# lez-s/Materialist

Measured on AMD Instinct MI355X. Metric: opt_iterations_per_sec_512x512, higher is better.
Workload: dtype f32; 1 GPU; BASELINE configs[1] synthetic: 1x512x512/GPU, --model_name pos_mlp --opt_order 'rm a' part rm, spp 64; mode=pos_mlp, height=512, width=512, spp=64, images_per_gpu=1, light=SH25, parallelism=dp1 (independent images, no data-path collective)

## Files before the change

### include/matpbr_mlp.h

```cpp
#ifndef MATPBR_MLP_H
#define MATPBR_MLP_H
#include <stddef.h>
#include <stdint.h>

#ifdef __cplusplus
extern "C" {
#endif

int matpbr_mlp_small_bwd_step(const float* g, int ldg, const float* w, int ldw, const float* c_prev, float* g_prev, int ldo, float* colsum_out,
                              int n_prev, const float* x, int ldx, float* d_w, int ldw_out, int K, const float* colsum_in, int colsum_stride,
                              int groups_in, float* d_bias, long M, int n_red, void* stream);

int matpbr_sin_bwd(const float* d_y, long ld_d, const float* pre, long ld_p, float* out, long M, int n, void* stream);
size_t matpbr_column_sum_workspace_bytes(int N);
int matpbr_column_sum(const float* x, float* out, long M, int N, void* workspace, size_t workspace_bytes, void* stream);

int matpbr_mlp_layer_fwd(const float* x, int ldx, const float* w, int ldw, const float* bias, float* s_out, float* c_out, int ldo, long M,
                         int N, int K, void* stream);
size_t matpbr_mlp_bwd_input_workspace_bytes(long M);
int matpbr_mlp_layer_bwd_input(const float* g, int ldg, const float* wt, int ldwt, const float* c_prev, float* g_prev, int ldo,
                               float* d_bias_prev, void* workspace, size_t workspace_bytes, long M, int n_prev, int n_red, void* stream);
size_t matpbr_mlp_bwd_weight_workspace_bytes(long M);
int matpbr_mlp_layer_bwd_weight(const float* g, int ldg, const float* x, int ldx, float* d_w, int ldw, void* workspace,
                                size_t workspace_bytes, long M, int N, int K, void* stream);
// ... 36 lines not shown
#define MATPBR_REDUCE_NONE (-1)
#define MATPBR_REDUCE_WGRAD 0
#define MATPBR_REDUCE_COLSUM 1
#define MATPBR_REDUCE_SKINNY 2
typedef struct MatpbrReduceJob {
    int kind, groups;
    const float *src, *src_b, *src_g;
    float *dst, *dst_b, *dst_g;
    int n0, n1, n2, n3;
    long ld_j, ld_c;
} MatpbrReduceJob;
int matpbr_mlp_reduce_jobs(const MatpbrReduceJob* jobs, int n_jobs, void* stream);
int matpbr_mlp_out_layer_bwd_tmax(const float* d_x, int ldd, const float* s_prev, const float* c_prev, int lds, const float* w_out, int ldw, float* g_prev,
                                  int ldg, void* g_tile_max, float* d_w, long ld_j, long ld_c, float* d_bias, float* d_bias_prev, void* workspace,
                                  size_t workspace_bytes, long M, int J, int n_prev, MatpbrReduceJob* defer, void* stream);
int matpbr_mlp_layer_bwd_input_blk(const float* g, int ldg, const void* g_tile_max, const void* wtsplit, const float* s_prev, float* g_prev, int ldo,
                                   void* out_tile_max, float* d_bias_prev, void* workspace, size_t workspace_bytes, long M, int n_prev, int n_red,
                                   MatpbrReduceJob* defer, void* stream);
int matpbr_mlp_first_layer_bwd_blk(const float* g, int ldg, const void* g_tile_max, const void* wtsplit, const float* s_prev, int lds, const float* x0,
                                   int ldx0, float* d_w0, long ld_j, long ld_c, int d0, float* d_bias0, void* workspace, size_t workspace_bytes,
                                   void* workspace2, size_t workspace2_bytes, long M, int n0, int n_red, MatpbrReduceJob* defer2, void* stream);
int matpbr_mlp_layer_bwd_weight_blk(const float* g, int ldg, const void* g_tile_max, const float* x, int ldx, float* d_w, int ldw, void* workspace,
                                    size_t workspace_bytes, long M, int N, int K, MatpbrReduceJob* defer, void* stream);
int matpbr_mlp_split_weights_multi(const float* const* w, const int* ldw, const int* N, const int* K, const int* transposed,
                                   void* const* wsplit, int n_jobs, void* stream);
int matpbr_mlp_skinny_fwd(const float* x, int ldx, const float* w, int ldw, const float* bias, float* out, int ldo, long M, int J, int K,
                          void* stream);
int matpbr_mlp_arm_head_fwd(const float* x, int ldx, const float* w, int ldw, const float* bias, const float* start, int lds, float* th,
                            float* map_a, float* map_r, float* map_m, long M, int K, void* stream);
int matpbr_mlp_arm_head_bwd(const float* g_a, const float* g_r, const float* g_m, const float* th, float* d_x, long M, void* stream);
size_t matpbr_mlp_skinny_workspace_bytes(int J);
int matpbr_mlp_out_layer_bwd(const float* d_x, int ldd, const float* s_prev, const float* c_prev, int lds, const float* w_out, int ldw, float* g_prev,
                             int ldg, float* d_w, long ld_j, long ld_c, float* d_bias, float* d_bias_prev, void* workspace, size_t workspace_bytes,
                             long M, int J, int n_prev, void* stream);
int matpbr_mlp_skinny_bwd_weight(const float* s, int lds, const float* b, int ldb, float* d_w, long ld_j, long ld_c, float* d_bias,
                                 void* workspace, size_t workspace_bytes, long M, int J, int C, void* stream);
int matpbr_adamw_step_dev(float* p, const float* g, float* m, float* v, long n, float* hyper, float beta1, float beta2, float eps,
                          float weight_decay, void* stream);
int matpbr_adamw_step_snapshot_dev(float* p, const float* g, float* m, float* v, long n, float* hyper, float beta1, float beta2,
                                   float eps, float weight_decay, float* best, const float* stats, void* stream);

#ifdef __cplusplus
}
#endif
#endif
```

### materialist_amd/_lib.py

```python
from __future__ import annotations

import ctypes
import os
import threading

from . import build as _build

_c_f = ctypes.c_void_p


class MatpbrCamera(ctypes.Structure):
    _fields_ = [("fov_x_deg", ctypes.c_float)]


class MatpbrBrdfPhase(ctypes.Structure):
    _fields_ = ([(k, ctypes.c_void_p) for k in ("pa", "pr", "pm", "n", "light", "gt_srgb", "a0", "r0", "m0", "dcache", "pred", "jac", "d_a",
                                                "d_r", "d_m")] +
                [("adam_m", ctypes.c_void_p * 3), ("adam_v", ctypes.c_void_p * 3)] +
                [(k, ctypes.c_void_p) for k in ("best_a", "best_r", "best_m", "best_img", "stats", "history", "workspace")] +
                [("workspace_bytes", ctypes.c_size_t), ("H", ctypes.c_int), ("W", ctypes.c_int), ("batch", ctypes.c_int), ("spp", ctypes.c_int),
                 ("fov_x_deg", ctypes.c_float), ("scale_delta", ctypes.c_float), ("part_mask", ctypes.c_uint32), ("es_patience", ctypes.c_int),
                 ("es_min_delta", ctypes.c_float), ("hist_len", ctypes.c_int), ("s1cache", ctypes.c_void_p), ("lazy_state", ctypes.c_void_p),
                 ("lazy_tol", ctypes.c_float), ("pred_next", ctypes.c_void_p), ("flags", ctypes.c_uint32), ("lazy_fold", ctypes.c_void_p)])

# ... 80 lines not shown
                                                 ctypes.c_size_t, ctypes.c_long, ctypes.c_int, ctypes.c_int, ctypes.c_void_p]),
    "matpbr_mlp_bwd_weight_workspace_bytes": (ctypes.c_size_t, [ctypes.c_long]),
    "matpbr_mlp_layer_bwd_weight": (ctypes.c_int, [_c_f, ctypes.c_int, _c_f, ctypes.c_int, _c_f, ctypes.c_int, ctypes.c_void_p, ctypes.c_size_t,
                                                  ctypes.c_long, ctypes.c_int, ctypes.c_int, ctypes.c_void_p]),
    "matpbr_mlp_layer_fwd_sgn": (ctypes.c_int, [_c_f, ctypes.c_int, _c_f, ctypes.c_int, _c_f, _c_f, ctypes.c_int, _c_f, ctypes.c_int, ctypes.c_long,
                                               ctypes.c_int, ctypes.c_int, ctypes.c_void_p]),
    "matpbr_mlp_layer_bwd_input_sgn": (ctypes.c_int, [_c_f, ctypes.c_int, _c_f, ctypes.c_int, _c_f, _c_f, ctypes.c_int, _c_f, ctypes.c_void_p,
                                                     ctypes.c_size_t, ctypes.c_long, ctypes.c_int, ctypes.c_int, ctypes.c_void_p]),
    "matpbr_mlp_layer_bwd_input_bx_sgn": (ctypes.c_int, [_c_f, ctypes.c_int, _c_f, _c_f, _c_f, ctypes.c_int, _c_f, ctypes.c_void_p, ctypes.c_size_t,
                                                        ctypes.c_long, ctypes.c_int, ctypes.c_int, ctypes.c_int, ctypes.c_void_p]),
    "matpbr_mlp_layer_bwd_weight_bx": (ctypes.c_int, [_c_f, ctypes.c_int, _c_f, ctypes.c_int, _c_f, ctypes.c_int, ctypes.c_void_p, ctypes.c_size_t,
                                                     ctypes.c_long, ctypes.c_int, ctypes.c_int, ctypes.c_int, ctypes.c_void_p]),
    "matpbr_mlp_out_layer_bwd_tmax": (ctypes.c_int, [_c_f, ctypes.c_int, _c_f, _c_f, ctypes.c_int, _c_f, ctypes.c_int, _c_f, ctypes.c_int, ctypes.c_void_p, _c_f,
                                                     ctypes.c_long, ctypes.c_long, _c_f, _c_f, ctypes.c_void_p, ctypes.c_size_t, ctypes.c_long, ctypes.c_int,
                                                     ctypes.c_int, ctypes.c_void_p, ctypes.c_void_p]),
    "matpbr_mlp_reduce_jobs": (ctypes.c_int, [ctypes.c_void_p, ctypes.c_int, ctypes.c_void_p]),
    "matpbr_mlp_layer_bwd_input_blk": (ctypes.c_int, [_c_f, ctypes.c_int, ctypes.c_void_p, ctypes.c_void_p, _c_f, _c_f, ctypes.c_int, ctypes.c_void_p, _c_f,
                                                      ctypes.c_void_p, ctypes.c_size_t, ctypes.c_long, ctypes.c_int, ctypes.c_int, ctypes.c_void_p, ctypes.c_void_p]),
    "matpbr_mlp_first_layer_bwd_blk": (ctypes.c_int, [_c_f, ctypes.c_int, ctypes.c_void_p, ctypes.c_void_p, _c_f, ctypes.c_int, _c_f, ctypes.c_int, _c_f,
                                                      ctypes.c_long, ctypes.c_long, ctypes.c_int, _c_f, ctypes.c_void_p, ctypes.c_size_t, ctypes.c_void_p,
                                                      ctypes.c_size_t, ctypes.c_long, ctypes.c_int, ctypes.c_int, ctypes.c_void_p, ctypes.c_void_p]),
    "matpbr_mlp_layer_bwd_weight_blk": (ctypes.c_int, [_c_f, ctypes.c_int, ctypes.c_void_p, _c_f, ctypes.c_int, _c_f, ctypes.c_int, ctypes.c_void_p,
                                                       ctypes.c_size_t, ctypes.c_long, ctypes.c_int, ctypes.c_int, ctypes.c_void_p, ctypes.c_void_p]),
    "matpbr_mlp_chain_images_bytes": (ctypes.c_size_t, []),
    "matpbr_mlp_chain_prep": (ctypes.c_int, [ctypes.c_void_p, ctypes.c_void_p, ctypes.c_void_p, ctypes.c_void_p, ctypes.c_int, ctypes.c_void_p, ctypes.c_void_p,
                                             ctypes.c_void_p, ctypes.c_long, ctypes.c_void_p]),
    "matpbr_mlp_chain_fwd": (ctypes.c_int, [_c_f, ctypes.c_int, ctypes.c_void_p, ctypes.c_void_p, ctypes.c_int, ctypes.c_void_p, _c_f, ctypes.c_int, _c_f, _c_f, _c_f,
                                            _c_f, ctypes.c_int, ctypes.c_long, ctypes.c_void_p]),
    "matpbr_mlp_split_weights_fmt": (ctypes.c_int, [_c_f, ctypes.c_int, ctypes.c_int, ctypes.c_int, ctypes.c_int, ctypes.c_void_p, ctypes.c_void_p]),
    "matpbr_mlp_skinny_fwd": (ctypes.c_int, [_c_f, ctypes.c_int, _c_f, ctypes.c_int, _c_f, _c_f, ctypes.c_int, ctypes.c_long, ctypes.c_int, ctypes.c_int,
                                            ctypes.c_void_p]),
    "matpbr_mlp_arm_head_fwd": (ctypes.c_int, [_c_f, ctypes.c_int, _c_f, ctypes.c_int, _c_f, _c_f, ctypes.c_int, _c_f, _c_f, _c_f, _c_f, ctypes.c_long,
                                              ctypes.c_int, ctypes.c_void_p]),
    "matpbr_mlp_arm_head_bwd": (ctypes.c_int, [_c_f, _c_f, _c_f, _c_f, _c_f, ctypes.c_long, ctypes.c_void_p]),
    "matpbr_mlp_skinny_workspace_bytes": (ctypes.c_size_t, [ctypes.c_int]),
    "matpbr_mlp_set_lds_dma": (ctypes.c_int, [ctypes.c_int]),
    "matpbr_mlp_skinny_bwd_weight": (ctypes.c_int, [_c_f, ctypes.c_int, _c_f, ctypes.c_int, _c_f, ctypes.c_long, ctypes.c_long, _c_f, ctypes.c_void_p,
                                                   ctypes.c_size_t, ctypes.c_long, ctypes.c_int, ctypes.c_int, ctypes.c_void_p]),
    "matpbr_adamw_step_dev": (ctypes.c_int, [_c_f] * 4 + [ctypes.c_long, _c_f, ctypes.c_float, ctypes.c_float, ctypes.c_float, ctypes.c_float,
                                                         ctypes.c_void_p]),
    "matpbr_light_to_sh25": (ctypes.c_int, [_c_f, ctypes.c_int, ctypes.c_int, _c_f, ctypes.c_int, ctypes.c_void_p]),
    "matpbr_light_to_sh25_bwd": (ctypes.c_int, [_c_f, ctypes.c_int, ctypes.c_int, _c_f, ctypes.c_int, ctypes.c_void_p]),
    "matpbr_mlp_split_weights_multi": (ctypes.c_int, [ctypes.c_void_p] * 6 + [ctypes.c_int, ctypes.c_void_p]),
    "matpbr_adamw_step_snapshot_dev": (ctypes.c_int, [_c_f] * 4 + [ctypes.c_long, _c_f, ctypes.c_float, ctypes.c_float, ctypes.c_float, ctypes.c_float,
                                                                  _c_f, _c_f, ctypes.c_void_p]),
    "matpbr_mlp_layer_fwd_tail": (ctypes.c_int, [_c_f, ctypes.c_int, _c_f, ctypes.c_int, _c_f, _c_f, _c_f, ctypes.c_int, _c_f, ctypes.c_int, ctypes.c_long,
# ... 76 lines not shown
```

### materialist_amd/csrc/posmlp_kernels.hip

```cpp
#include <hip/hip_runtime.h>
#include <stdint.h>
#include <atomic>
#include <type_traits>

#include "../../include/matpbr.h"
#include "../../include/matpbr_experimental.h"
#include "posmlp_device.hpp"

namespace {


constexpr int kBM = 128, kBN = 128, kBK = 32;
constexpr int kPersistent = 512;
constexpr int EPI_SINCOS = 0, EPI_MULC = 1, EPI_BIAS = 2;

struct HeadArgs {
  const float* w;
  int ldw;
  const float* bias;
  ArmHead h;
};

__global__ __launch_bounds__(256) void mlp_tail_copy_kernel(float* __restrict__ out, int ldo, const float* __restrict__ tail, int ldt, long M, int N) {
  const int w = 256 - N;
// ... 1435 lines not shown
                                                                    acc[mi][ni], 0, 0, 0);
          }
        }
        if (s == 0) asm volatile("s_waitcnt vmcnt(4) lgkmcnt(0)\n\ts_barrier" ::: "memory");
        else asm volatile("s_waitcnt vmcnt(0) lgkmcnt(0)\n\ts_barrier" ::: "memory");
        wb ^= 1;
      }
      ab ^= 1;
    }
    float* scr = reinterpret_cast<float*>(gx_smem + (size_t)(wb ^ 1) * kGxW + wave * 6144);
    float* sW4 = reinterpret_cast<float*>(gx_smem + 2 * kGxW + (size_t)(ab ^ 1) * kGlRows);
    float* sComb = sW4 + 5 * 256;
    const int t_row = lane >> 3, t_col = (lane & 7) * 4;
    if (HEAD) {
      for (int i = tid; i < 5 * 256; i += kGxThreads) sW4[i] = hd.w[(size_t)(i >> 8) * hd.ldw + (i & 255)];
      __syncthreads();
    }
    float* sx = reinterpret_cast<float*>(gx_smem + 2 * kGxW + (size_t)(ab ^ 1) * kGlRows + wave * 4096);
    if (W0) {
      const float* xs = p.x0 + (size_t)(row0 + wm * 64 + lane) * p.ldx0;
#pragma unroll
      for (int q = 0; q < 4; ++q) *reinterpret_cast<float4*>(sx + lane * 16 + 4 * ((q + lane) & 3)) = *reinterpret_cast<const float4*>(xs + 4 * ((q + lane) & 3));
    }
    float4 cvb[2][4];
    auto cv_load = [&](int b, float4 (&dst)[4]) {
      const float* src = p.cmul + (size_t)(row0 + wm * 64 + (b >> 2) * 32 + t_row) * p.ldo + wn * 128 + (b & 3) * 32 + t_col;
#pragma unroll
      for (int ps = 0; ps < 4; ++ps) dst[ps] = *reinterpret_cast<const float4*>(src + (size_t)(8 * ps) * p.ldo);
    };
    if (EPI == EPI_MULC) cv_load(0, cvb[0]);
    float hacc[4][5];
#pragma unroll
    for (int b = 0; b < 8; ++b) {
      const int mi = b >> 2, ni = b & 3;
      const size_t o0 = (size_t)(row0 + wm * 64 + mi * 32 + t_row) * p.ldo + wn * 128 + ni * 32 + t_col;
      if (EPI == EPI_MULC && b + 1 < 8) cv_load(b + 1, cvb[(b + 1) & 1]);
      if (HEAD && ni == 0) {
#pragma unroll
        for (int ps = 0; ps < 4; ++ps)
#pragma unroll
          for (int j = 0; j < 5; ++j) hacc[ps][j] = 0.f;
      }
      float second[16];
#pragma unroll
      for (int r = 0; r < 16; ++r) {
        float v = acc[mi][ni][r];
        if (BLK) v *= a_unscale;
        if (EPI == EPI_SINCOS) {
          const float pre = F16 ? __builtin_fmaf(v, kF16WUnscale, bn[ni]) : v + bn[ni];
          if (PK) v = sin_packed(pre);
          else sincos_cw(pre, v, second[r]);
        }
        scr[((r & 3) + 8 * (r >> 2) + 4 * lh) * kLd + li] = v;
      }
      float4 vrow[4];
#pragma unroll
      for (int ps = 0; ps < 4; ++ps) {
        float4 v = *reinterpret_cast<const float4*>(scr + (t_row + 8 * ps) * kLd + t_col);
        if (EPI == EPI_MULC) {
          float4 c4 = cvb[b & 1][ps];
          if (p.cmul_sin) c4 = cos_from_packed_sin(c4);
          v.x *= c4.x; v.y *= c4.y; v.z *= c4.z; v.w *= c4.w;
          csum4[ni].x += v.x; csum4[ni].y += v.y; csum4[ni].z += v.z; csum4[ni].w += v.w;
          if (BLK && !W0) omax = __builtin_fmaxf(__builtin_fmaxf(omax, __builtin_fmaxf(__builtin_fabsf(v.x), __builtin_fabsf(v.y))),
                                                   __builtin_fmaxf(__builtin_fabsf(v.z), __builtin_fabsf(v.w)));
        }
        if (EPI == EPI_SINCOS && !HEAD && ni == 3 && p.tail != nullptr && wn == 1) {
            const int col = 224 + t_col;
            const float* tl = p.tail + (size_t)(row0 + wm * 64 + mi * 32 + t_row + 8 * ps) * p.ldt - p.N;
            if (col >= p.N) v.x = tl[col];
            if (col + 1 >= p.N) v.y = tl[col + 1];
            if (col + 2 >= p.N) v.z = tl[col + 2];
            if (col + 3 >= p.N) v.w = tl[col + 3];
        }
        if (W0) *reinterpret_cast<float4*>(scr + (t_row + 8 * ps) * kLd + t_col) = v;
        else *reinterpret_cast<float4*>(p.out0 + o0 + (size_t)(8 * ps) * p.ldo) = v;
        vrow[ps] = v;
      }
      if (W0) {
#pragma unroll
        for (int ct = 0; ct < 2; ++ct)
#pragma unroll
          for (int kk = 0; kk < 8; ++kk)
            acc0[ni][ct] = __builtin_amdgcn_mfma_f32_16x16x4f32(scr[(4 * kk + (lane >> 4)) * kLd + 16 * ct + (lane & 15)],
                                                                sx[(mi * 32 + 4 * kk + (lane >> 4)) * 16 + (lane & 15)], acc0[ni][ct], 0, 0, 0);
      }
      if (HEAD) {
#pragma unroll
        for (int j = 0; j < 5; ++j) {
          const float4 w4 = *reinterpret_cast<const float4*>(sW4 + j * 256 + wn * 128 + ni * 32 + t_col);
#pragma unroll
          for (int ps = 0; ps < 4; ++ps)
            hacc[ps][j] = __builtin_fmaf(vrow[ps].x, w4.x, __builtin_fmaf(vrow[ps].y, w4.y, __builtin_fmaf(vrow[ps].z, w4.z, __builtin_fmaf(vrow[ps].w, w4.w, hacc[ps][j]))));
        }
      }
      if (EPI == EPI_SINCOS && !PK) {
#pragma unroll
        for (int r = 0; r < 16; ++r) scr[((r & 3) + 8 * (r >> 2) + 4 * lh) * kLd + li] = second[r];
#pragma unroll
        for (int ps = 0; ps < 4; ++ps)
          *reinterpret_cast<float4*>(p.out1 + o0 + (size_t)(8 * ps) * p.ldo) = *reinterpret_cast<const float4*>(scr + (t_row + 8 * ps) * kLd + t_col);
      }
      if (HEAD && ni == 3) {
#pragma unroll
        for (int ps = 0; ps < 4; ++ps)
#pragma unroll
          for (int j = 0; j < 5; ++j) {
            float v = hacc[ps][j];
// ... 43 lines not shown
#pragma unroll
    for (int sl = 0; sl < 16; ++sl) t += sRed[sl * 256 + tid];
    p.colsum[(size_t)blockIdx.x * 256 + tid] = t;
  }
}

constexpr int kWgStage = 2 * 3 * 2 * 256;
constexpr size_t kWgSmem = 2 * kWgStage * sizeof(uint4);
#ifndef MATPBR_WG_DEPTH
#define MATPBR_WG_DEPTH 2
#endif
constexpr int kWgDepth = MATPBR_WG_DEPTH;
constexpr int kWgThreads = 512;
__device__ __forceinline__ int wg_perm(int i) { return (i & 16) + 2 * (i & 7) + ((i >> 3) & 1); }
template <int NPROD, bool EARLY>
__device__ __forceinline__ void wgrad_bx_body(const float* __restrict__ G, int ldg, const float* __restrict__ X, int ldx,
                                              float* __restrict__ partial, long M, long rows_per_slab, uint4* sW, const unsigned* __restrict__ g_tmax) {
  constexpr bool F16 = NPROD == 3;
  constexpr int NP = F16 ? 2 : 3;
  const int tid = threadIdx.x, lane = tid & 63, wave = tid >> 6;
  const int nq = wave >> 1, kq = wave & 1, li = lane & 31, lh = lane >> 5;
  const long m_begin = (long)blockIdx.x * rows_per_slab;
  const long m_end = (m_begin + rows_per_slab < M) ? m_begin + rows_per_slab : M;
  const int steps = m_begin < m_end ? (int)((m_end - m_begin) / 16) : 0;
  float g_scale = 1.0f, g_unscale = 1.0f;
  if (F16 && steps > 0) {
    unsigned mb = 0;
    for (long t = m_begin / kBM; t <= (m_end - 1) / kBM; ++t) mb = g_tmax[t] > mb ? g_tmax[t] : mb;
    block_scale(mb, g_scale, g_unscale);
  }

  f32x16 acc[2][4];
#pragma unroll
  for (int ni = 0; ni < 2; ++ni)
#pragma unroll
    for (int ki = 0; ki < 4; ++ki)
#pragma unroll
      for (int r = 0; r < 16; ++r) acc[ni][ki][r] = 0.f;

  const int cp = tid & 255, sh = tid >> 8;
  const float* src = (cp >> 7) ? X + (m_begin + 8 * sh) * ldx + 2 * (cp & 127) : G + (m_begin + 8 * sh) * ldg + 2 * (cp & 127);
  const long ld = (cp >> 7) ? ldx : ldg;
  const float my_scale = (F16 && !(cp >> 7)) ? g_scale : 1.0f;
  uint4* sdst = sW + (((cp >> 7) * NP) * 2 + sh) * 256 + ((cp & 127) >> 3) * 16 + (cp & 7);
  float2 raw[kWgDepth][8];
  auto load_stage = [&](int slot, int step) {
#pragma unroll
    for (int j = 0; j < 8; ++j) raw[slot][j] = *reinterpret_cast<const float2*>(src + (16L * step + j) * ld);
  };
  auto split_store = [&](int slot, int buf) {
#pragma unroll
    for (int c = 0; c < 2; ++c) {
      uint4 pc[3];
      const float2* r = raw[slot];
#define MATPBR_COMP(v) (c == 0 ? (v).x : (v).y)
      if (F16) {
        split2h(MATPBR_COMP(r[0]) * my_scale, MATPBR_COMP(r[1]) * my_scale, pc[0].x, pc[1].x);
        split2h(MATPBR_COMP(r[2]) * my_scale, MATPBR_COMP(r[3]) * my_scale, pc[0].y, pc[1].y);
        split2h(MATPBR_COMP(r[4]) * my_scale, MATPBR_COMP(r[5]) * my_scale, pc[0].z, pc[1].z);
        split2h(MATPBR_COMP(r[6]) * my_scale, MATPBR_COMP(r[7]) * my_scale, pc[0].w, pc[1].w);
      } else {
        split3(MATPBR_COMP(r[0]), MATPBR_COMP(r[1]), pc[0].x, pc[1].x, pc[2].x);
        split3(MATPBR_COMP(r[2]), MATPBR_COMP(r[3]), pc[0].y, pc[1].y, pc[2].y);
        split3(MATPBR_COMP(r[4]), MATPBR_COMP(r[5]), pc[0].z, pc[1].z, pc[2].z);
        split3(MATPBR_COMP(r[6]), MATPBR_COMP(r[7]), pc[0].w, pc[1].w, pc[2].w);
      }
#undef MATPBR_COMP
#pragma unroll
      for (int piece = 0; piece < NP; ++piece) sdst[buf * kWgStage + (piece * 2) * 256 + 8 * c] = pc[piece];
    }
  };
// ... 80 lines not shown
      for (int r = 0; r < 16; ++r) {
        const int n = nq * 64 + ni * 32 + wg_perm((r & 3) + 8 * (r >> 2) + 4 * lh);
        const int k = kq * 128 + ki * 32 + wg_perm(li);
        out[n * 256 + k] = F16 ? acc[ni][ki][r] * g_unscale : acc[ni][ki][r];
      }
}

template <int NPROD>
__global__ __launch_bounds__(kWgThreads, 1) void mlp_wgrad_bx(const float* __restrict__ G, int ldg, const float* __restrict__ X, int ldx,
                                                              float* __restrict__ partial, long M, long rows_per_slab, const unsigned* __restrict__ g_tmax) {
  extern __shared__ __align__(16) unsigned char wg_smem[];
  uint4* sW = reinterpret_cast<uint4*>(wg_smem);
  if (threadIdx.x >> 8)
    wgrad_bx_body<NPROD, true>(G, ldg, X, ldx, partial, M, rows_per_slab, sW, g_tmax);
  else
    wgrad_bx_body<NPROD, false>(G, ldg, X, ldx, partial, M, rows_per_slab, sW, g_tmax);
}

#ifndef MATPBR_WG_HX
#define MATPBR_WG_HX 1
#endif
constexpr int kHxRaw = 16 * 2 * 1024;
constexpr int kHxPieces = 2 * 2 * 2 * 256;
constexpr size_t kHxSmem = 3 * kHxRaw + kHxPieces * sizeof(uint4);
__global__ __launch_bounds__(kWgThreads, 1) void mlp_wgrad_hx(const float* __restrict__ G, int ldg, const float* __restrict__ X, int ldx,
                                                              float* __restrict__ partial, long M, long rows_per_slab, const unsigned* __restrict__ g_tmax) {
  extern __shared__ __align__(16) unsigned char hx_smem[];
  uint4* sP = reinterpret_cast<uint4*>(hx_smem + 3 * kHxRaw);
  const int tid = threadIdx.x, lane = tid & 63, wave = tid >> 6;
  const int nq = wave >> 1, kq = wave & 1, li = lane & 31, lh = lane >> 5;
  (void)rows_per_slab;
  const int tiles = (int)(M / kBM);
  const int t_first = tiles - 1 - (int)blockIdx.x;
  const int my_tiles = t_first >= 0 ? t_first / (int)gridDim.x + 1 : 0;
  const int steps = my_tiles * (kBM / 16);
  float g_scale = 1.0f, g_unscale = 1.0f;
  if (steps > 0) {
    unsigned mb = 0;
    for (int t = t_first; t >= 0; t -= (int)gridDim.x) mb = g_tmax[t] > mb ? g_tmax[t] : mb;
    block_scale(mb, g_scale, g_unscale);
  }
  f32x16 acc[2][4];
#pragma unroll
  for (int ni = 0; ni < 2; ++ni)
#pragma unroll
    for (int ki = 0; ki < 4; ++ki)
#pragma unroll
// ... 4 lines not shown
    const unsigned lds0 = lds_byte_address(hx_smem);
    unsigned vg[4], vx[4];
#pragma unroll
    for (int j = 0; j < 4; ++j) {
      vg[j] = (unsigned)(j * ldg) * 4u + (unsigned)lane * 16u - 1024u * j;
      vx[j] = (unsigned)(j * ldx) * 4u + (unsigned)lane * 16u - 1024u * j;
    }
    auto issue = [&](int step, int buf) {
      const int sc = step < steps ? step : steps - 1;
      const long row = ((long)t_first - (long)(sc >> 3) * gridDim.x) * kBM + 16 * (7 - (sc & 7)) + 4 * wave_u;
      const unsigned dst = lds0 + (unsigned)buf * (unsigned)kHxRaw + (unsigned)wave_u * 4096u;
      glds16_x4v(G + row * ldg, vg[0], vg[1], vg[2], vg[3], dst);
      glds16_x4v(X + row * ldx, vx[0], vx[1], vx[2], vx[3], dst + 16u * 1024u);
    };
    const int cp = tid & 255, sh = tid >> 8;
    const float my_scale = (cp >> 7) ? 1.0f : g_scale;
    const unsigned raw_off = (unsigned)((cp >> 7) * 16 * 1024 + (8 * sh) * 1024 + (cp & 127) * 8);
    uint4* sdst = sP + (((cp >> 7) * 2) * 2 + sh) * 256 + ((cp & 127) >> 3) * 16 + (cp & 7);
    float2 raw[8];
    auto read_raw = [&](int buf) {
#pragma unroll
      for (int j = 0; j < 8; ++j) raw[j] = *reinterpret_cast<const float2*>(hx_smem + buf * kHxRaw + raw_off + j * 1024);
    };
    auto cut_store = [&]() {
#pragma unroll
      for (int c = 0; c < 2; ++c) {
        uint4 pc[2];
#define MATPBR_COMP(v) (c == 0 ? (v).x : (v).y)
        split2h(MATPBR_COMP(raw[0]) * my_scale, MATPBR_COMP(raw[1]) * my_scale, pc[0].x, pc[1].x);
        split2h(MATPBR_COMP(raw[2]) * my_scale, MATPBR_COMP(raw[3]) * my_scale, pc[0].y, pc[1].y);
        split2h(MATPBR_COMP(raw[4]) * my_scale, MATPBR_COMP(raw[5]) * my_scale, pc[0].z, pc[1].z);
        split2h(MATPBR_COMP(raw[6]) * my_scale, MATPBR_COMP(raw[7]) * my_scale, pc[0].w, pc[1].w);
#undef MATPBR_COMP
#pragma unroll
        for (int piece = 0; piece < 2; ++piece) sdst[(piece * 2) * 256 + 8 * c] = pc[piece];
      }
    };
    auto products = [&](const uint4 (&a)[2][2], const uint4 (&b)[2][4]) {
#pragma unroll
      for (int ki = 0; ki < 4; ++ki)
#pragma unroll
        for (int t = 0; t < 3; ++t) {
          constexpr int ia[3] = {1, 0, 0}, ib[3] = {0, 1, 0};
#pragma unroll
          for (int ni = 0; ni < 2; ++ni)
            acc[ni][ki] = __builtin_amdgcn_mfma_f32_32x32x16_f16(__builtin_bit_cast(f16x8, a[ia[t]][ni]), __builtin_bit_cast(f16x8, b[ib[t]][ki]), acc[ni][ki], 0, 0, 0);
        }
    };
    if (loader) { issue(0, 0); issue(1, 1); }
    if (loader) asm volatile("s_waitcnt vmcnt(8)" ::: "memory");
    asm volatile("s_barrier" ::: "memory");
    read_raw(0);
    cut_store();
    if (loader) issue(2, 2);
    const uint4* sa = sP + lh * 256 + nq * 64 + li;
    const uint4* sb = sP + (2 * 2 + lh) * 256 + kq * 128 + li;
    int nxt = 1;
    for (int st = 0; st < steps; ++st) {
      if (loader) asm volatile("s_waitcnt vmcnt(8)" ::: "memory");
      asm volatile("s_waitcnt lgkmcnt(0)\n\ts_barrier" ::: "memory");
      uint4 a[2][2], b[2][4];
#pragma unroll
      for (int piece = 0; piece < 2; ++piece) {
#pragma unroll
        for (int ni = 0; ni < 2; ++ni) a[piece][ni] = sa[(piece * 2) * 256 + ni * 32];
#pragma unroll
        for (int ki = 0; ki < 4; ++ki) b[piece][ki] = sb[(piece * 2) * 256 + ki * 32];
      }
      read_raw(nxt);
      asm volatile("s_waitcnt lgkmcnt(0)\n\ts_barrier" ::: "memory");
      if (loader) {
        issue(st + 3, nxt == 0 ? 2 : nxt - 1);
        __builtin_amdgcn_sched_barrier(0);
      }
      products(a, b);
      cut_store();
      nxt = nxt == 2 ? 0 : nxt + 1;
    }
    asm volatile("s_waitcnt vmcnt(0)" ::: "memory");
  }
  float* out = partial + (long)blockIdx.x * 256 * 256;
#pragma unroll
  for (int ni = 0; ni < 2; ++ni)
#pragma unroll
    for (int ki = 0; ki < 4; ++ki)
#pragma unroll
      for (int r = 0; r < 16; ++r) {
        const int n = nq * 64 + ni * 32 + wg_perm((r & 3) + 8 * (r >> 2) + 4 * lh);
        const int k = kq * 128 + ki * 32 + wg_perm(li);
        out[n * 256 + k] = acc[ni][ki][r] * g_unscale;
      }
}

constexpr size_t kBxSmem = 2 * kBxStage * sizeof(uint4) + 8 * 32 * kLd * sizeof(float);
constexpr size_t kBxSmemHead = kBxSmem + (5 * 256 + 128 * 2 * 8) * sizeof(float);
std::atomic<int> g_nt_gl{2};
std::atomic<int> g_nt_w0_gx{0};
inline bool gl_ok(const NtArgs& p) {
  return g_nt_gl.load(std::memory_order_relaxed) != 0 && p.K > 32 && (long)kBM * p.lda * 4 < (1l << 31);
}
template <auto Kernel>
bool lds_opt_in(size_t bytes) {
  static std::atomic<unsigned long long> done{0};
  int dev = 0;
  if (hipGetDevice(&dev) != hipSuccess) return false;
  const unsigned long long bit = 1ull << (dev & 63);
  if (done.load(std::memory_order_acquire) & bit) return true;
  if (hipFuncSetAttribute(reinterpret_cast<const void*>(Kernel), hipFuncAttributeMaxDynamicSharedMemorySize, (int)bytes) != hipSuccess) return false;
  done.fetch_or(bit, std::memory_order_release);
  return true;
}
template <int EPI, int NPROD, bool FULL>
bool launch_nt_bx_full(const NtArgs& p, const uint4* wsplit, unsigned grid, hipStream_t stream) {
  if constexpr (FULL) if (gl_ok(p)) {
    if (!lds_opt_in<&mlp_nt_bx<EPI, NPROD, true, false, false, true>>(kGlSmem)) return false;
    hipLaunchKernelGGL((mlp_nt_bx<EPI, NPROD, true, false, false, true>), dim3(grid), dim3(kBxThreads), kGlSmem, stream, p, wsplit, HeadArgs{});
    return true;
  }
  if (!lds_opt_in<&mlp_nt_bx<EPI, NPROD, FULL>>(kBxSmem)) return false;
  hipLaunchKernelGGL((mlp_nt_bx<EPI, NPROD, FULL>), dim3(grid), dim3(kBxThreads), kBxSmem, stream, p, wsplit, HeadArgs{});
// ... 500 lines not shown
  if (q.kind == MATPBR_REDUCE_WGRAD) wgrad_reduce_body(red, q.src, q.groups, q.dst, q.n0, q.n1, q.n2, block);
  else if (q.kind == MATPBR_REDUCE_COLSUM) colsum_reduce_body(red, q.src, q.groups, q.dst, block);
  else skinny_reduce_body(red, block, q.src, q.src_b, q.groups, q.n0, q.n1, q.n2, q.dst, q.ld_j, q.ld_c, q.dst_b, q.src_g, q.n3, q.dst_g);
}
inline int reduce_job_blocks(const MatpbrReduceJob& q) {
  if (q.kind == MATPBR_REDUCE_WGRAD) return 256;
  if (q.kind == MATPBR_REDUCE_COLSUM) return q.n0;
  return q.n0 * 4 + (q.dst_g ? 4 : 0);
}
inline void launch_reduce_job(const MatpbrReduceJob& q, hipStream_t st) {
  if (q.kind == MATPBR_REDUCE_WGRAD) hipLaunchKernelGGL(mlp_wgrad_reduce, dim3(256), dim3(1024), 0, st, q.src, q.groups, q.dst, q.n0, q.n1, q.n2);
  else if (q.kind == MATPBR_REDUCE_COLSUM) hipLaunchKernelGGL(mlp_colsum_reduce, dim3(q.n0), dim3(256), 0, st, q.src, q.groups, q.dst);
  else hipLaunchKernelGGL(mlp_skinny_tn_reduce, dim3(reduce_job_blocks(q)), dim3(1024), 0, st, q.src, q.src_b, q.groups, q.n0, q.n1, q.n2, q.dst, q.ld_j, q.ld_c,
                          q.dst_b, q.src_g, q.n3, q.dst_g);
}
inline void reduce_or_defer(const MatpbrReduceJob& q, MatpbrReduceJob* defer, hipStream_t st) {
  if (defer) *defer = q;
  else launch_reduce_job(q, st);
}

}

extern "C" {

int matpbr_mlp_set_lds_dma(int mode) {
  g_nt_w0_gx.store(mode == 3 ? 1 : 0, std::memory_order_relaxed);
  const int was = g_nt_gl.exchange(mode < 0 ? 0 : (mode > 2 ? 2 : mode), std::memory_order_relaxed);
  return was;
}

int matpbr_mlp_layer_fwd_tail(const float* x, int ldx, const float* w, int ldw, const float* bias, float* s_out, float* c_out, int ldo,
                              const float* tail, int ldt, long M, int N, int K, void* stream) {
  if (!x || !w || !bias || !s_out || M <= 0 || M > 0x7fffff00L || N <= 0 || N > 256 || K <= 0 || K > 256) return MATPBR_ERR_INVALID_ARG;
  if ((ldx & 3) || (ldw & 3) || ldx < ((K + 3) & ~3) || ldw < ((K + 3) & ~3) || ldo < N || !aligned16(x) || !aligned16(w))
    return MATPBR_ERR_INVALID_ARG;
  if (tail && (ldo < 256 || ldt < 256 - N || !c_out)) return MATPBR_ERR_INVALID_ARG;
  NtArgs p{x, w, bias, nullptr, s_out, c_out, nullptr, 0, N, K, ldx, ldw, ldo};
  p.tail = tail; p.ldt = ldt;
  const bool thin = M > kSmallM && K <= 16 && ldx >= thin_pad(K) && ldw >= ((K + 3) & ~3) && ldo >= 256 && !(ldo & 3) && aligned16(s_out) &&
                    (!c_out || aligned16(c_out));
  if (M <= kSmallM) {
    if (c_out) launch_small_nt<EPI_SINCOS>(p, M, (hipStream_t)stream);
    else launch_small_nt<EPI_BIAS>(p, M, (hipStream_t)stream);
  } else if (thin) {
    p.M = (int)M;
    if (c_out) launch_thin_k<EPI_SINCOS>(p, (hipStream_t)stream);
// ... 292 lines not shown
    hipLaunchKernelGGL(mlp_small_tn, dim3((unsigned)tiles), dim3(256), 0, (hipStream_t)stream, g, ldg, x, ldx, d_w, ldw, (int)M, N, K);
    return hipGetLastError() == hipSuccess ? MATPBR_OK : MATPBR_ERR_LAUNCH;
  }
  if (!workspace || workspace_bytes < matpbr_mlp_bwd_weight_workspace_bytes(M)) return MATPBR_ERR_WORKSPACE;
  const int slabs = wgrad_slabs(M);
  long rows = (M + slabs - 1) / slabs;
  rows = (rows + kWM - 1) / kWM * kWM;
  hipLaunchKernelGGL(mlp_wgrad_tn, dim3(slabs, (N + 127) / 128), dim3(256), 0, (hipStream_t)stream, g, ldg, x, ldx, (float*)workspace, M, rows, K);
  hipLaunchKernelGGL(mlp_wgrad_reduce, dim3(256), dim3(1024), 0, (hipStream_t)stream, (const float*)workspace, slabs, d_w, N, K, ldw);
  return hipGetLastError() == hipSuccess ? MATPBR_OK : MATPBR_ERR_LAUNCH;
}

static int mlp_layer_bwd_weight_bx_impl(const float* g, int ldg, const float* x, int ldx, float* d_w, int ldw, void* workspace,
                                        size_t workspace_bytes, long M, int N, int K, int nprod, const unsigned* g_tile_max, void* stream,
                                        MatpbrReduceJob* defer = nullptr) {
  if (!g || !x || !d_w || M <= 0 || N <= 0 || N > 256 || K <= 0 || K > 256) return MATPBR_ERR_INVALID_ARG;
  if (nprod == 3 && (!g_tile_max || (M % kBM))) return MATPBR_ERR_INVALID_ARG;
  if ((nprod != 3 && nprod != 6 && nprod != 9) || (M & 15) || ldg < 256 || ldx < 256 || (ldg & 3) || (ldx & 3) || ldw < K || !aligned16(g) || !aligned16(x))
    return MATPBR_ERR_UNSUPPORTED;
  if (!workspace || workspace_bytes < matpbr_mlp_bwd_weight_workspace_bytes(M)) return MATPBR_ERR_WORKSPACE;
  int slabs = wgrad_slabs(M);
  long rows = ((M + slabs - 1) / slabs + 15) / 16 * 16;
  slabs = (int)((M + rows - 1) / rows);
  if (nprod == 3 && MATPBR_WG_HX && (long)ldg * 4 >= 1024 && (long)ldx * 4 >= 1024 && (long)3 * ldg * 4 + 1024 < (1l << 31) && (long)3 * ldx * 4 + 1024 < (1l << 31)) {
    if (!lds_opt_in<&mlp_wgrad_hx>(kHxSmem)) return MATPBR_ERR_LAUNCH;
    hipLaunchKernelGGL(mlp_wgrad_hx, dim3(slabs), dim3(kWgThreads), kHxSmem, (hipStream_t)stream, g, ldg, x, ldx, (float*)workspace, M, rows, g_tile_max);
  } else if (nprod == 3) {
    if (!lds_opt_in<&mlp_wgrad_bx<3>>(kWgSmem)) return MATPBR_ERR_LAUNCH;
    hipLaunchKernelGGL(mlp_wgrad_bx<3>, dim3(slabs), dim3(kWgThreads), kWgSmem, (hipStream_t)stream, g, ldg, x, ldx, (float*)workspace, M, rows, g_tile_max);
  } else if (nprod == 6) {
    if (!lds_opt_in<&mlp_wgrad_bx<6>>(kWgSmem)) return MATPBR_ERR_LAUNCH;
    hipLaunchKernelGGL(mlp_wgrad_bx<6>, dim3(slabs), dim3(kWgThreads), kWgSmem, (hipStream_t)stream, g, ldg, x, ldx, (float*)workspace, M, rows, (const unsigned*)nullptr);
  } else {
    if (!lds_opt_in<&mlp_wgrad_bx<9>>(kWgSmem)) return MATPBR_ERR_LAUNCH;
    hipLaunchKernelGGL(mlp_wgrad_bx<9>, dim3(slabs), dim3(kWgThreads), kWgSmem, (hipStream_t)stream, g, ldg, x, ldx, (float*)workspace, M, rows, (const unsigned*)nullptr);
  }
  MatpbrReduceJob q{};
  q.kind = MATPBR_REDUCE_WGRAD; q.groups = slabs; q.src = (const float*)workspace; q.dst = d_w; q.n0 = N; q.n1 = K; q.n2 = ldw;
  reduce_or_defer(q, defer, (hipStream_t)stream);
  return hipGetLastError() == hipSuccess ? MATPBR_OK : MATPBR_ERR_LAUNCH;
}
int matpbr_mlp_layer_bwd_weight_bx(const float* g, int ldg, const float* x, int ldx, float* d_w, int ldw, void* workspace,
                                   size_t workspace_bytes, long M, int N, int K, int nprod, void* stream) {
  if (nprod == 3) return MATPBR_ERR_INVALID_ARG;
  return mlp_layer_bwd_weight_bx_impl(g, ldg, x, ldx, d_w, ldw, workspace, workspace_bytes, M, N, K, nprod, nullptr, stream);
}
int matpbr_mlp_layer_bwd_weight_blk(const float* g, int ldg, const void* g_tile_max, const float* x, int ldx, float* d_w, int ldw, void* workspace,
// ... 113 lines not shown
```

### materialist_amd/ops.py

```python
from __future__ import annotations

import ctypes
from typing import Dict, Optional

import torch

from . import _lib
from ._lib import MatpbrCamera, MatpbrError

LIGHT_SH25 = 0
NSH = 25
MAX_SPP = 128
FLAG_CLAMP_PARAMS = 1
FLAG_ATTACHED_SAMPLING = 2
FLAG_LAZY_FORCE = 16
FLAG_JAC16 = 32
FLAG_MODELS_READY = 64
FLAG_ROTATE_BEST = 128
FLAG_GENERIC_STEP = 256
FLAG_JAC32 = 512
FLAG_SHARE_GPU = 2048
LAZY_NSTATE = 28
LAZY_PLANES = 30
STATS_STRIDE = 16
# ... 787 lines not shown
    ws = _mlp_workspace("bwd_input" + (defer[1] if defer else ""), M, g.device, lib.matpbr_mlp_bwd_input_workspace_bytes(M))
    ws2 = _mlp_workspace("skinny2" + (defer[1] if defer else ""), 0, g.device, lib.matpbr_mlp_skinny_workspace_bytes(16))
    with torch.cuda.device(g.device):
        code = lib.matpbr_mlp_first_layer_bwd_blk(_ptr(g), g.stride(0), _ptr(g_tile_max), _ptr(wtsplit), _ptr(s_prev), s_prev.stride(0), _ptr(x0), x0.stride(0),
                                                  _ptr(d_w0), 1, d_w0.stride(0), int(d0), _ptr(d_bias0), _ptr(ws), ws.numel() * 4, _ptr(ws2), ws2.numel() * 4,
                                                  M, int(n0), int(n_red), defer[0] if defer else None, _stream(g))
    _lib.check(code, "matpbr_mlp_first_layer_bwd_blk")


def mlp_layer_bwd_weight_blk(g: torch.Tensor, g_tile_max: torch.Tensor, x: torch.Tensor, N: int, K: int, out: Optional[torch.Tensor] = None,
                             defer=None) -> torch.Tensor:
    lib = _lib.load()
    g, x = _mat2(g, "g"), _mat2(x, "x")
    M = g.shape[0]
    ws = _mlp_workspace("bwd_weight" + (defer[1] if defer else ""), M, g.device, lib.matpbr_mlp_bwd_weight_workspace_bytes(M))
    d_w = out if out is not None else torch.empty((N, K), dtype=torch.float32, device=g.device)
    with torch.cuda.device(g.device):
        code = lib.matpbr_mlp_layer_bwd_weight_blk(_ptr(g), g.stride(0), _ptr(g_tile_max), _ptr(x), x.stride(0), _ptr(d_w), d_w.stride(0), _ptr(ws),
                                                   ws.numel() * 4, M, N, K, defer[0] if defer else None, _stream(g))
    _lib.check(code, "matpbr_mlp_layer_bwd_weight_blk")
    return d_w


def mlp_reduce_jobs(jobs, n: int, like: torch.Tensor) -> None:
    with torch.cuda.device(like.device):
        code = _lib.load().matpbr_mlp_reduce_jobs(ctypes.byref(jobs), int(n), _stream(like))
    _lib.check(code, "matpbr_mlp_reduce_jobs")


LIGHT_SH9, LIGHT_ENV_TEXELS = 1, 2


class _LightToSh25(torch.autograd.Function):
    @staticmethod
    def forward(ctx, light, kind):
        lib = _lib.load()
        light = _dev(light, "light")
        B, n = light.shape[0], light.shape[1]
        out = torch.empty((B, NSH, 3), dtype=torch.float32, device=light.device)
        with torch.cuda.device(light.device):
            code = lib.matpbr_light_to_sh25(_ptr(light), int(kind), n, _ptr(out), B, _stream(light))
        _lib.check(code, "matpbr_light_to_sh25")
        ctx.kind, ctx.n = int(kind), n
        return out

    @staticmethod
# ... 36 lines not shown
```

Baseline: 643.0 it/s.

## Double-buffer wgrad_hx pieces, reorder F16 wgrad tile walk, trim W0 prefetch

The half-precision wgrad kernel gets a second LDS piece buffer and a deeper three-stage global prefetch. Loader waves and compute waves now run separate loops so fragment reads and products overlap with the next cut/store. The F16 blocked wgrad kernel walks tiles in a strided reverse order instead of contiguous slabs, so its reads match the per-tile max layout. The W0 epilogue uses a single cv buffer, moves the prefetch next to the MFMA loop and adds sched barriers. A runtime switch for the hx kernel is also added. The larger LDS footprint and the split barrier sequences between loader and compute waves add risk of deadlock or lower occupancy.

New measurement: 650.2 it/s (median of 6 runs). +1.1%, better.

```diff
diff --git a/include/matpbr_mlp.h b/include/matpbr_mlp.h
--- a/include/matpbr_mlp.h
+++ b/include/matpbr_mlp.h
@@ -82,6 +82,7 @@
                                    void* workspace2, size_t workspace2_bytes, long M, int n0, int n_red, MatpbrReduceJob* defer2, void* stream);
 int matpbr_mlp_layer_bwd_weight_blk(const float* g, int ldg, const void* g_tile_max, const float* x, int ldx, float* d_w, int ldw, void* workspace,
                                     size_t workspace_bytes, long M, int N, int K, MatpbrReduceJob* defer, void* stream);
+int matpbr_mlp_set_wgrad_kernel(int kernel);
 int matpbr_mlp_split_weights_multi(const float* const* w, const int* ldw, const int* N, const int* K, const int* transposed,
                                    void* const* wsplit, int n_jobs, void* stream);
 int matpbr_mlp_skinny_fwd(const float* x, int ldx, const float* w, int ldw, const float* bias, float* out, int ldo, long M, int J, int K,
diff --git a/materialist_amd/_lib.py b/materialist_amd/_lib.py
--- a/materialist_amd/_lib.py
+++ b/materialist_amd/_lib.py
@@ -126,6 +126,7 @@
                                                       ctypes.c_size_t, ctypes.c_long, ctypes.c_int, ctypes.c_int, ctypes.c_void_p, ctypes.c_void_p]),
     "matpbr_mlp_layer_bwd_weight_blk": (ctypes.c_int, [_c_f, ctypes.c_int, ctypes.c_void_p, _c_f, ctypes.c_int, _c_f, ctypes.c_int, ctypes.c_void_p,
                                                        ctypes.c_size_t, ctypes.c_long, ctypes.c_int, ctypes.c_int, ctypes.c_void_p, ctypes.c_void_p]),
+    "matpbr_mlp_set_wgrad_kernel": (ctypes.c_int, [ctypes.c_int]),
     "matpbr_mlp_chain_images_bytes": (ctypes.c_size_t, []),
     "matpbr_mlp_chain_prep": (ctypes.c_int, [ctypes.c_void_p, ctypes.c_void_p, ctypes.c_void_p, ctypes.c_void_p, ctypes.c_int, ctypes.c_void_p, ctypes.c_void_p,
                                              ctypes.c_void_p, ctypes.c_long, ctypes.c_void_p]),
diff --git a/materialist_amd/csrc/posmlp_kernels.hip b/materialist_amd/csrc/posmlp_kernels.hip
--- a/materialist_amd/csrc/posmlp_kernels.hip
+++ b/materialist_amd/csrc/posmlp_kernels.hip
@@ -1481,7 +1481,8 @@
 #pragma unroll
       for (int q = 0; q < 4; ++q) *reinterpret_cast<float4*>(sx + lane * 16 + 4 * ((q + lane) & 3)) = *reinterpret_cast<const float4*>(xs + 4 * ((q + lane) & 3));
     }
-    float4 cvb[2][4];
+    constexpr int kCvSets = W0 ? 1 : 2;
+    float4 cvb[kCvSets][4];
     auto cv_load = [&](int b, float4 (&dst)[4]) {
       const float* src = p.cmul + (size_t)(row0 + wm * 64 + (b >> 2) * 32 + t_row) * p.ldo + wn * 128 + (b & 3) * 32 + t_col;
 #pragma unroll
@@ -1493,7 +1494,7 @@
     for (int b = 0; b < 8; ++b) {
       const int mi = b >> 2, ni = b & 3;
       const size_t o0 = (size_t)(row0 + wm * 64 + mi * 32 + t_row) * p.ldo + wn * 128 + ni * 32 + t_col;
-      if (EPI == EPI_MULC && b + 1 < 8) cv_load(b + 1, cvb[(b + 1) & 1]);
+      if (EPI == EPI_MULC && !W0 && b + 1 < 8) cv_load(b + 1, cvb[(b + 1) & (kCvSets - 1)]);
       if (HEAD && ni == 0) {
 #pragma unroll
         for (int ps = 0; ps < 4; ++ps)
@@ -1517,7 +1518,7 @@
       for (int ps = 0; ps < 4; ++ps) {
         float4 v = *reinterpret_cast<const float4*>(scr + (t_row + 8 * ps) * kLd + t_col);
         if (EPI == EPI_MULC) {
-          float4 c4 = cvb[b & 1][ps];
+          float4 c4 = cvb[b & (kCvSets - 1)][ps];
           if (p.cmul_sin) c4 = cos_from_packed_sin(c4);
           v.x *= c4.x; v.y *= c4.y; v.z *= c4.z; v.w *= c4.w;
           csum4[ni].x += v.x; csum4[ni].y += v.y; csum4[ni].z += v.z; csum4[ni].w += v.w;
@@ -1537,12 +1538,15 @@
         vrow[ps] = v;
       }
       if (W0) {
-#pragma unroll
-        for (int ct = 0; ct < 2; ++ct)
+        if (EPI == EPI_MULC && b + 1 < 8) cv_load(b + 1, cvb[0]);
+#pragma unroll
+        for (int ct = 0; ct < 2; ++ct) {
 #pragma unroll
           for (int kk = 0; kk < 8; ++kk)
             acc0[ni][ct] = __builtin_amdgcn_mfma_f32_16x16x4f32(scr[(4 * kk + (lane >> 4)) * kLd + 16 * ct + (lane & 15)],
                                                                 sx[(mi * 32 + 4 * kk + (lane >> 4)) * 16 + (lane & 15)], acc0[ni][ct], 0, 0, 0);
+          __builtin_amdgcn_sched_barrier(0);
+        }
       }
       if (HEAD) {
 #pragma unroll
@@ -1632,11 +1636,15 @@
   const int nq = wave >> 1, kq = wave & 1, li = lane & 31, lh = lane >> 5;
   const long m_begin = (long)blockIdx.x * rows_per_slab;
   const long m_end = (m_begin + rows_per_slab < M) ? m_begin + rows_per_slab : M;
-  const int steps = m_begin < m_end ? (int)((m_end - m_begin) / 16) : 0;
+  const int t_first = F16 ? (int)(M / kBM) - 1 - (int)blockIdx.x : 0;
+  const int steps = F16 ? (t_first >= 0 ? (t_first / (int)gridDim.x + 1) * (kBM / 16) : 0) : (m_begin < m_end ? (int)((m_end - m_begin) / 16) : 0);
+  auto step_row = [&](int step) -> long {
+    return F16 ? ((long)t_first - (long)(step >> 3) * gridDim.x) * kBM + 16 * (7 - (step & 7)) : m_begin + 16L * step;
+  };
   float g_scale = 1.0f, g_unscale = 1.0f;
   if (F16 && steps > 0) {
     unsigned mb = 0;
-    for (long t = m_begin / kBM; t <= (m_end - 1) / kBM; ++t) mb = g_tmax[t] > mb ? g_tmax[t] : mb;
+    for (int t = t_first; t >= 0; t -= (int)gridDim.x) mb = g_tmax[t] > mb ? g_tmax[t] : mb;
     block_scale(mb, g_scale, g_unscale);
   }
 
@@ -1649,14 +1657,14 @@
       for (int r = 0; r < 16; ++r) acc[ni][ki][r] = 0.f;
 
   const int cp = tid & 255, sh = tid >> 8;
-  const float* src = (cp >> 7) ? X + (m_begin + 8 * sh) * ldx + 2 * (cp & 127) : G + (m_begin + 8 * sh) * ldg + 2 * (cp & 127);
+  const float* src = (cp >> 7) ? X + (8 * sh) * (long)ldx + 2 * (cp & 127) : G + (8 * sh) * (long)ldg + 2 * (cp & 127);
   const long ld = (cp >> 7) ? ldx : ldg;
   const float my_scale = (F16 && !(cp >> 7)) ? g_scale : 1.0f;
   uint4* sdst = sW + (((cp >> 7) * NP) * 2 + sh) * 256 + ((cp & 127) >> 3) * 16 + (cp & 7);
   float2 raw[kWgDepth][8];
   auto load_stage = [&](int slot, int step) {
 #pragma unroll
-    for (int j = 0; j < 8; ++j) raw[slot][j] = *reinterpret_cast<const float2*>(src + (16L * step + j) * ld);
+    for (int j = 0; j < 8; ++j) raw[slot][j] = *reinterpret_cast<const float2*>(src + (step_row(step) + j) * ld);
   };
   auto split_store = [&](int slot, int buf) {
 #pragma unroll
@@ -1783,7 +1791,8 @@
 #endif
 constexpr int kHxRaw = 16 * 2 * 1024;
 constexpr int kHxPieces = 2 * 2 * 2 * 256;
-constexpr size_t kHxSmem = 3 * kHxRaw + kHxPieces * sizeof(uint4);
+constexpr size_t kHxSmem = 3 * kHxRaw + 2 * kHxPieces * sizeof(uint4);
+static_assert(kHxSmem <= 160 * 1024, "mlp_wgrad_hx: the LDS of a CU");
 __global__ __launch_bounds__(kWgThreads, 1) void mlp_wgrad_hx(const float* __restrict__ G, int ldg, const float* __restrict__ X, int ldx,
                                                               float* __restrict__ partial, long M, long rows_per_slab, const unsigned* __restrict__ g_tmax) {
   extern __shared__ __align__(16) unsigned char hx_smem[];
@@ -1834,7 +1843,7 @@
 #pragma unroll
       for (int j = 0; j < 8; ++j) raw[j] = *reinterpret_cast<const float2*>(hx_smem + buf * kHxRaw + raw_off + j * 1024);
     };
-    auto cut_store = [&]() {
+    auto cut_store = [&](int pb) {
 #pragma unroll
       for (int c = 0; c < 2; ++c) {
         uint4 pc[2];
@@ -1845,7 +1854,18 @@
         split2h(MATPBR_COMP(raw[6]) * my_scale, MATPBR_COMP(raw[7]) * my_scale, pc[0].w, pc[1].w);
 #undef MATPBR_COMP
 #pragma unroll
-        for (int piece = 0; piece < 2; ++piece) sdst[(piece * 2) * 256 + 8 * c] = pc[piece];
+        for (int piece = 0; piece < 2; ++piece) sdst[pb * kHxPieces + (piece * 2) * 256 + 8 * c] = pc[piece];
+      }
+    };
+    const uint4* sa = sP + lh * 256 + nq * 64 + li;
+    const uint4* sb = sP + (2 * 2 + lh) * 256 + kq * 128 + li;
+    auto read_frags = [&](int pb, uint4 (&a)[2][2], uint4 (&b)[2][4]) {
+#pragma unroll
+      for (int piece = 0; piece < 2; ++piece) {
+#pragma unroll
+        for (int ni = 0; ni < 2; ++ni) a[piece][ni] = sa[pb * kHxPieces + (piece * 2) * 256 + ni * 32];
+#pragma unroll
+        for (int ki = 0; ki < 4; ++ki) b[piece][ki] = sb[pb * kHxPieces + (piece * 2) * 256 + ki * 32];
       }
     };
     auto products = [&](const uint4 (&a)[2][2], const uint4 (&b)[2][4]) {
@@ -1859,36 +1879,46 @@
             acc[ni][ki] = __builtin_amdgcn_mfma_f32_32x32x16_f16(__builtin_bit_cast(f16x8, a[ia[t]][ni]), __builtin_bit_cast(f16x8, b[ib[t]][ki]), acc[ni][ki], 0, 0, 0);
         }
     };
-    if (loader) { issue(0, 0); issue(1, 1); }
-    if (loader) asm volatile("s_waitcnt vmcnt(8)" ::: "memory");
+#define MATPBR_HX_BARRIER() do { __builtin_amdgcn_sched_barrier(0); asm volatile("s_waitcnt lgkmcnt(0)\n\ts_barrier" ::: "memory"); __builtin_amdgcn_sched_barrier(0); } while (0)
+    if (loader) { issue(0, 0); issue(1, 1); issue(2, 2); }
+    if (loader) asm volatile("s_waitcnt vmcnt(16)" ::: "memory");
     asm volatile("s_barrier" ::: "memory");
     read_raw(0);
-    cut_store();
-    if (loader) issue(2, 2);
-    const uint4* sa = sP + lh * 256 + nq * 64 + li;
-    const uint4* sb = sP + (2 * 2 + lh) * 256 + kq * 128 + li;
+    cut_store(0);
+    uint4 a[2][2], b[2][4];
     int nxt = 1;
-    for (int st = 0; st < steps; ++st) {
-      if (loader) asm volatile("s_waitcnt vmcnt(8)" ::: "memory");
-      asm volatile("s_waitcnt lgkmcnt(0)\n\ts_barrier" ::: "memory");
-      uint4 a[2][2], b[2][4];
-#pragma unroll
-      for (int piece = 0; piece < 2; ++piece) {
-#pragma unroll
-        for (int ni = 0; ni < 2; ++ni) a[piece][ni] = sa[(piece * 2) * 256 + ni * 32];
-#pragma unroll
-        for (int ki = 0; ki < 4; ++ki) b[piece][ki] = sb[(piece * 2) * 256 + ki * 32];
-      }
-      read_raw(nxt);
-      asm volatile("s_waitcnt lgkmcnt(0)\n\ts_barrier" ::: "memory");
-      if (loader) {
+    if (loader) {
+      for (int st = 0; st < steps; ++st) {
+        asm volatile("s_waitcnt vmcnt(8)" ::: "memory");
+        MATPBR_HX_BARRIER();
         issue(st + 3, nxt == 0 ? 2 : nxt - 1);
         __builtin_amdgcn_sched_barrier(0);
+        read_frags(st & 1, a, b);
+        read_raw(nxt);
+        cut_store((st + 1) & 1);
+        MATPBR_HX_BARRIER();
+        products(a, b);
+        nxt = nxt == 2 ? 0 : nxt + 1;
+      }
+    } else {
+      MATPBR_HX_BARRIER();
+      MATPBR_HX_BARRIER();
+      read_frags(0, a, b);
+      read_raw(1);
+      cut_store(1);
+      nxt = 2;
+      for (int st = 1; st < steps; ++st) {
+        MATPBR_HX_BARRIER();
+        products(a, b);
+        MATPBR_HX_BARRIER();
+        read_frags(st & 1, a, b);
+        read_raw(nxt);
+        cut_store((st + 1) & 1);
+        nxt = nxt == 2 ? 0 : nxt + 1;
       }
       products(a, b);
-      cut_store();
-      nxt = nxt == 2 ? 0 : nxt + 1;
-    }
+    }
+#undef MATPBR_HX_BARRIER
     asm volatile("s_waitcnt vmcnt(0)" ::: "memory");
   }
   float* out = partial + (long)blockIdx.x * 256 * 256;
@@ -1908,6 +1938,7 @@
 constexpr size_t kBxSmemHead = kBxSmem + (5 * 256 + 128 * 2 * 8) * sizeof(float);
 std::atomic<int> g_nt_gl{2};
 std::atomic<int> g_nt_w0_gx{0};
+std::atomic<int> g_wg_hx{MATPBR_WG_HX};
 inline bool gl_ok(const NtArgs& p) {
   return g_nt_gl.load(std::memory_order_relaxed) != 0 && p.K > 32 && (long)kBM * p.lda * 4 < (1l << 31);
 }
@@ -2454,6 +2485,8 @@
 }
 
 extern "C" {
+
+int matpbr_mlp_set_wgrad_kernel(int kernel) { return g_wg_hx.exchange(kernel != 0 ? 1 : 0, std::memory_order_relaxed); }
 
 int matpbr_mlp_set_lds_dma(int mode) {
   g_nt_w0_gx.store(mode == 3 ? 1 : 0, std::memory_order_relaxed);
@@ -2792,7 +2825,7 @@
   int slabs = wgrad_slabs(M);
   long rows = ((M + slabs - 1) / slabs + 15) / 16 * 16;
   slabs = (int)((M + rows - 1) / rows);
-  if (nprod == 3 && MATPBR_WG_HX && (long)ldg * 4 >= 1024 && (long)ldx * 4 >= 1024 && (long)3 * ldg * 4 + 1024 < (1l << 31) && (long)3 * ldx * 4 + 1024 < (1l << 31)) {
+  if (nprod == 3 && g_wg_hx.load(std::memory_order_relaxed) != 0 && (long)ldg * 4 >= 1024 && (long)ldx * 4 >= 1024 && (long)3 * ldg * 4 + 1024 < (1l << 31) && (long)3 * ldx * 4 + 1024 < (1l << 31)) {
     if (!lds_opt_in<&mlp_wgrad_hx>(kHxSmem)) return MATPBR_ERR_LAUNCH;
     hipLaunchKernelGGL(mlp_wgrad_hx, dim3(slabs), dim3(kWgThreads), kHxSmem, (hipStream_t)stream, g, ldg, x, ldx, (float*)workspace, M, rows, g_tile_max);
   } else if (nprod == 3) {
diff --git a/materialist_amd/ops.py b/materialist_amd/ops.py
--- a/materialist_amd/ops.py
+++ b/materialist_amd/ops.py
@@ -833,6 +833,10 @@
     return d_w
 
 
+def mlp_set_wgrad_kernel(kernel: int) -> int:
+    return int(_lib.load().matpbr_mlp_set_wgrad_kernel(int(kernel)))
+
+
 def mlp_reduce_jobs(jobs, n: int, like: torch.Tensor) -> None:
     with torch.cuda.device(like.device):
         code = _lib.load().matpbr_mlp_reduce_jobs(ctypes.byref(jobs), int(n), _stream(like))
```
